# Funatiq/cuclark

Hardware: AMD Instinct MI355X
Metric: Mreads/sec (10M x 150bp, k=31) (higher is better)
Workload: dtype u64

## Files before the change

### cuclark_amd/_lib.py

```python
import ctypes as C
import importlib.util
import os
import subprocess

_PKG = os.path.dirname(os.path.abspath(__file__))
LIB_PATH = os.environ.get("MIC_LIB_PATH") or os.path.join(_PKG, "lib", "libmi_clark.so")
CSRC = os.path.join(_PKG, "csrc")

MIC_RESULT_WORDS = 8
MIC_FLAG_ROW_OVERFLOW = 1
MIC_FLAG_DENSE_PATH = 2
MIC_ROW_INVALID = 0xFFFFFFFF
MIC_ROLLUP_WORDS, MIC_ROLLUP_MAX_LEVELS = 8, 7
MIC_ROLLUP_UNRESOLVED, MIC_ROLLUP_PENDING = 0xFFFFFFFF, 0xFFFFFFFE
MIC_DENSITY_WORDS, MIC_DENSITY_CONF_BINS, MIC_DENSITY_GAMMA_BINS = 5153, 51, 101
MIC_KSKETCH_REGS = 16384
MIC_LAYOUT_AUTO, MIC_LAYOUT_DIRECT, MIC_LAYOUT_MINIMIZER, MIC_LAYOUT_SUPER, MIC_LAYOUT_SUPER2 = 0, 1, 2, 3, 4


class MicError(RuntimeError):
    def __init__(self, code, msg):
        super().__init__(f"libmi_clark error {code}: {msg}")
        self.code = code

# ... 63 lines not shown
    ("mic_batch_query_group", C.c_int, [C.POINTER(C.c_void_p), _SZ, _SZ, C.c_int]),
    ("mic_sync", C.c_int, [_VP]),
    ("mic_thread_bind_near_device", C.c_int, [_VP, C.c_int]),
    ("mic_batches_free", C.c_int, [_VP]),
    ("mic_query_device", C.c_int, [_VP, _VP, _VP, _SZ, _VP, _VP, _VP]),
    ("mic_resolve_flagged_device", C.c_int, [_VP, _VP, _VP, _VP, _VP, _VP, C.POINTER(_SZ)]),
    ("mic_merge_rows_device", C.c_int, [_VP, _VP, _VP, _VP, _SZ, _VP]),
    ("mic_result_from_rows_device", C.c_int, [_VP, _VP, _VP, _SZ, _VP]),
    ("mic_count_dense_device", C.c_int, [_VP, _VP, _VP, _VP, _SZ, _VP, _VP]),
    ("mic_result_from_dense_device", C.c_int, [_VP, _VP, _VP, _SZ, _VP, _VP, _VP]),
    ("mic_probe_stats_device", C.c_int, [_VP, _VP, _VP, _SZ, C.POINTER(C.c_uint64)]),
    ("mic_last_query_ms", C.c_int, [_VP, C.POINTER(C.c_float)]),
    ("mic_last_crowd_stats", C.c_int, [_VP, C.POINTER(C.c_uint32)]),
    ("mic_debug_fetch_crowd", C.c_int, [_VP, _VP, _SZ, C.POINTER(C.c_uint32)]),
    ("mic_debug_fetch_slots", C.c_int, [_VP, C.c_uint64, C.c_uint64, _VP]),
    ("mic_debug_stream_pool", C.c_int, [C.POINTER(C.c_uint32)]),
    ("mic_ingest_alloc", C.c_int, [_VP, _SZ, _SZ, C.POINTER(C.c_char_p), C.c_uint32, C.c_int, C.POINTER(_VP)]),
    ("mic_ingest_classify", C.c_int, [_VP, _SZ, _SZ, C.c_int, C.POINTER(MicIngestResult)]),
    ("mic_ingest_classify_group", C.c_int, [C.POINTER(C.c_void_p), _SZ, _SZ, _SZ, _SZ, C.c_int, C.POINTER(MicIngestResult)]),
    ("mic_ingest_fetch_group_rows", C.c_int, [_VP, _SZ, _SZ, _VP, _SZ, C.POINTER(C.c_uint64), C.POINTER(C.c_uint32)]),
    ("mic_ingest_group_stats", C.c_int, [_VP, C.POINTER(C.c_double), _SZ]),
    ("mic_ingest_fetch_packed", C.c_int, [_VP, _SZ, _VP, _SZ, _VP, _SZ, C.POINTER(C.c_uint64), C.POINTER(C.c_uint64)]),
    ("mic_ingest_free", C.c_int, [_VP]),
    ("mic_ingest_set_min_quality", C.c_int, [_VP, C.c_uint32]),
    ("mic_fastq_mask_quality", C.c_int, [_VP, _SZ, C.c_uint32, _VP]),
    ("mic_ingest_set_low_complexity", C.c_int, [_VP, C.c_uint32]),
    ("mic_text_mask_low_complexity", C.c_int, [_VP, _SZ, C.c_uint32, _VP]),
    ("mic_gz_inflate_device", C.c_int, [_VP, _VP, _SZ, C.POINTER(_VP), C.POINTER(_SZ), C.POINTER(C.c_uint32)]),
    ("mic_gz_copy_text", C.c_int, [_VP, _VP, _SZ, _SZ, _VP]),
    ("mic_gz_free_text", C.c_int, [_VP, _VP]),
# ... 141 lines not shown
```

### cuclark_amd/csrc/mic_build.hip

```cpp
#include "mic_internal.h"
#include "mic_device.h"

#include <stdio.h>
#include <stdlib.h>
#include <time.h>
#include <vector>
#include <math.h>

#include <hipcub/hipcub.hpp>

#define TILE 256

namespace {

struct TileA { unsigned long long elems; unsigned long long nonzero; };
struct TileB { unsigned long long ovf_slots; unsigned long long kept; unsigned int max_bucket; unsigned int pad; };

__device__ inline void block_scan2(uint32_t a, uint32_t b, uint32_t& ex_a, uint32_t& ex_b, uint32_t& tot_a,
                                   uint32_t& tot_b) {
  __shared__ uint32_t sa[TILE], sb[TILE];
  const int t = threadIdx.x;
  sa[t] = a; sb[t] = b;
  __syncthreads();
  for (int off = 1; off < TILE; off <<= 1) {
// ... 672 lines not shown
__device__ inline uint64_t s_x_of(unsigned long long K, uint32_t j, int k, int m) {
  return (K >> (2 * (k - m - (int)j))) & ((1ULL << (2 * m)) - 1);
}
__device__ inline bool s_less(unsigned long long Ka, uint32_t ma, unsigned long long Kb, uint32_t mb, int k, int m) {
  const uint64_t xa = s_x_of(Ka, ma & 0xFF, k, m), xb = s_x_of(Kb, mb & 0xFF, k, m);
  if ((uint32_t)xa != (uint32_t)xb) return (uint32_t)xa < (uint32_t)xb;
  if (xa != xb) return xa < xb;
  return (ma & 0xFF) < (mb & 0xFF);
}

struct SWriter {
  uint32_t* slots; uint64_t main, chain; uint32_t n_total, n_out;
  uint64_t cur, n_slots; uint32_t n_here, pool_cap; uint32_t* pool; bool full;
  uint32_t row[32];
  __device__ __forceinline__ void row_init() {
    row[0] = row[1] = row[2] = row[3] = row[4] = row[5] = 0xFFFFFFFFu;
    row[6] = row[7] = row[8] = row[9] = row[10] = row[11] = row[12] = row[13] = row[14] = row[15] = row[16] = row[17] = row[18] = 0;
    row[19] = row[20] = row[21] = row[22] = row[23] = row[24] = row[25] = row[26] = row[27] = row[28] = row[29] = row[30] = row[31] = 0;
  }
#define S_ROW_PUT(ee) { const bool h_ = e == ee; row[ee] = h_ ? key : row[ee]; row[6 + 3 * ee] = h_ ? a : row[6 + 3 * ee]; row[7 + 3 * ee] = h_ ? b : row[7 + 3 * ee]; \
                        row[8 + 3 * ee] = h_ ? c : row[8 + 3 * ee]; row[24 + ee] = h_ ? pl : row[24 + ee]; }
  __device__ __forceinline__ void put_main(uint32_t e, uint32_t key, uint32_t a, uint32_t b, uint32_t c, uint32_t pl) {
    static_assert(MIC_S_CAP == 6, "one S_ROW_PUT per entry of a slot");
    S_ROW_PUT(0) S_ROW_PUT(1) S_ROW_PUT(2) S_ROW_PUT(3) S_ROW_PUT(4) S_ROW_PUT(5)
  }
#undef S_ROW_PUT
  __device__ __forceinline__ void put(uint64_t slot, uint32_t e, uint32_t key, uint32_t a, uint32_t b, uint32_t c, uint32_t pl) {
    if (slot == main) put_main(e, key, a, b, c, pl);
    else { uint32_t* q = slots + slot * 32; q[e] = key; q[6 + 3 * e] = a; q[7 + 3 * e] = b; q[8 + 3 * e] = c; q[24 + e] = pl; }
  }
  __device__ __forceinline__ void set_hdr(uint64_t slot, uint32_t w30, uint32_t w31) {
    if (slot == main) { row[30] = w30; row[31] = w31; } else { uint32_t* q = slots + slot * 32; q[30] = w30; q[31] = w31; }
  }
};

__device__ inline void s_slot_init(uint32_t* q) {
  for (int e = 0; e < 6; ++e) q[e] = 0xFFFFFFFFu;
  for (int e = 6; e < 32; ++e) q[e] = 0;
}
template <int MODE>
__device__ __forceinline__ void s_emit(const SOpen& o, uint64_t x, int L, SWriter& wr) {
  const u128 v = o.S << (96 - 2 * L);
  const uint32_t v0 = (uint32_t)(v >> 64), v1 = (uint32_t)(v >> 32), v2 = (uint32_t)v, pl = (o.pmask << 16) | o.label;
  if (MODE == 2) {
    if (wr.n_here == MIC_S_CAP && !wr.full) {
      const uint32_t idx = atomicAdd(wr.pool, 1u);
      if (idx >= wr.pool_cap) { wr.full = true; atomicMax(wr.pool + 1, 1u); }
      else {
        const uint64_t nxt = wr.n_slots + idx;
        wr.set_hdr(wr.cur, MIC_S_CAP | MIC_S_NEXT, (uint32_t)nxt);
        s_slot_init(wr.slots + nxt * 32);
        wr.cur = nxt; wr.n_here = 0;
      }
    }
    if (!wr.full) wr.put(wr.cur, wr.n_here++, (uint32_t)x, v0, v1, v2, pl);
  }
  if (MODE == 1) {
    const uint32_t idx = wr.n_out, e = idx % MIC_S_CAP;
    if (idx < MIC_S_CAP) wr.put_main(e, (uint32_t)x, v0, v1, v2, pl);
    else { uint32_t* q = wr.slots + (wr.chain + (idx - MIC_S_CAP) / MIC_S_CAP) * 32; q[e] = (uint32_t)x; q[6 + 3 * e] = v0; q[7 + 3 * e] = v1; q[8 + 3 * e] = v2; q[24 + e] = pl; }
  }
  ++wr.n_out;
}

#define S_MAXOPEN 4
#define S_TPB 128
#define S_LDS_CAND 2048
template <int MODE>
__global__ void __launch_bounds__(S_TPB) s_merge_kernel(const unsigned long long* __restrict__ off, const uint32_t* __restrict__ cnt,
                                                        uint64_t n_slots, unsigned long long* __restrict__ cand_k,
                                                        uint32_t* __restrict__ cand_m, int k, int m,
                                                        uint32_t* __restrict__ n_ent, const unsigned long long* __restrict__ chain_off,
                                                        uint32_t* __restrict__ slots, uint32_t* __restrict__ max_ent,
                                                        uint64_t slot_lo, uint64_t slot_hi, unsigned long long base, int sort_now,
                                                        uint32_t* __restrict__ pool, uint32_t pool_cap) {
// ... 29 lines not shown
    kv = (r + 2 * m >= 64 ? 0ULL : left << (r + 2 * m)) | (x << r) | ((unsigned long long)F & ((1ULL << r) - 1));
  };
  const uint32_t n = live ? cnt[s] : 0;
  const unsigned long long my = live ? off[s] - base : c0;
  const int w = k - m + 1, L = k + w - 1;
  SWriter wr; wr.slots = slots; wr.main = s; wr.chain = 0; wr.n_total = 0; wr.n_out = 0;
  wr.cur = s; wr.n_slots = n_slots; wr.n_here = 0; wr.pool_cap = pool_cap; wr.pool = pool; wr.full = false;
  wr.row_init();
  if (WRITE && live) {
    wr.n_total = n_ent[s];
    const uint32_t n_chain = wr.n_total > MIC_S_CAP ? (wr.n_total - 1) / MIC_S_CAP : 0;
    wr.chain = n_slots + chain_off[s];
    for (uint32_t c = 0; c <= n_chain; ++c) {
      const uint32_t here = wr.n_total - c * MIC_S_CAP > MIC_S_CAP ? MIC_S_CAP : wr.n_total - c * MIC_S_CAP;
      const uint32_t w30 = (wr.n_total ? here : 0) | (c < n_chain ? MIC_S_NEXT : 0), w31 = c < n_chain ? (uint32_t)(wr.chain + c) : 0;
      if (c == 0) { wr.row[30] = w30; wr.row[31] = w31; }
      else { uint32_t* q = slots + (wr.chain + c - 1) * 32; s_slot_init(q); q[30] = w30; q[31] = w31; }
    }
  }
  auto sort_and_merge = [&](auto* K, auto* M) __attribute__((always_inline)) {
  if (sort_now) {
    constexpr uint32_t gaps[8] = {701, 301, 132, 57, 23, 10, 4, 1};
#pragma unroll
    for (int g = 0; g < 8; ++g) {
      const uint32_t gap = gaps[g];
      if (gap >= n) continue;
      for (uint32_t i = gap; i < n; ++i) {
        const unsigned long long kv = K[i]; const uint32_t mv = M[i];
        uint32_t j = i;
        while (j >= gap && (packed ? kv < K[j - gap] : s_less(kv, mv, K[j - gap], M[j - gap], k, m))) { K[j] = K[j - gap]; M[j] = M[j - gap]; j -= gap; }
        K[j] = kv; M[j] = mv;
      }
// ... 56 lines not shown
#undef S_ROW_OUT
  }
}

__global__ void s_chain_demand_kernel(const uint32_t* __restrict__ n_ent, uint64_t n, uint32_t* __restrict__ demand) {
  uint64_t i = (uint64_t)blockIdx.x * blockDim.x + threadIdx.x;
  if (i < n) { const uint32_t e = n_ent[i]; demand[i] = e > MIC_S_CAP ? (e - 1) / MIC_S_CAP : 0; }
}

#ifndef MIC_S_CROWD
#define MIC_S_CROWD 12
#endif

struct SChain {
  const uint32_t* slots; uint64_t slot; uint32_t e, n_here; bool valid;
  __device__ SChain(const uint32_t* sl, uint64_t s) : slots(sl), slot(s), e(0) { n_here = sl[s * 32 + 30] & 0xFFu; valid = true; settle(); }
  __device__ void settle() {
    while (valid && e >= n_here) {
      const uint32_t* q = slots + slot * 32;
      if (q[30] & MIC_S_NEXT) { slot = q[31]; n_here = slots[slot * 32 + 30] & 0xFFu; e = 0; } else valid = false;
    }
  }
  __device__ void next() { ++e; settle(); }
  __device__ const uint32_t* q() const { return slots + slot * 32; }
};

__device__ inline uint64_t s_entry_x(const uint32_t* q, uint32_t e, int k, int m) {
  const u128 S = ((u128)q[6 + 3 * e] << 64) | ((u128)q[7 + 3 * e] << 32) | q[8 + 3 * e];
  const int ctx = k - m;
  return (uint64_t)(S >> (96 - 2 * (ctx + m))) & ((1ULL << (2 * m)) - 1);
}

__global__ void __launch_bounds__(256) s_crowd_count_kernel(const uint32_t* __restrict__ slots, uint64_t slot_lo, uint64_t slot_hi, int k, int m,
                                                            unsigned long long* __restrict__ out) {
  const uint64_t s = slot_lo + (uint64_t)blockIdx.x * blockDim.x + threadIdx.x;
  if (s >= slot_hi) return;
  if ((slots[s * 32 + 30] & 0xFFu) < MIC_S_CAP || !(slots[s * 32 + 30] & MIC_S_NEXT)) return;
  SChain c(slots, s);
  while (c.valid) {
    const uint64_t x = s_entry_x(c.q(), c.e, k, m);
    uint32_t n = 0, kmers = 0;
    while (c.valid && s_entry_x(c.q(), c.e, k, m) == x) { ++n; kmers += __popc(c.q()[24 + c.e] >> 16); c.next(); }
    if (n > MIC_S_CROWD) { atomicAdd(&out[0], (unsigned long long)kmers); atomicAdd(&out[1], 1ull); }
  }
}

__device__ inline void s_side_insert(uint4* __restrict__ side, uint32_t mask, uint64_t K, uint32_t label1) {
  uint32_t h = s_side_hash(K, mask);
  for (;;) {
    uint32_t* cell = (uint32_t*)(side + h);
    if (atomicCAS(&cell[2], 0u, label1) == 0u) { cell[0] = (uint32_t)K; cell[1] = (uint32_t)(K >> 32); return; }
    h = (h + 1) & mask;
  }
}

__global__ void __launch_bounds__(256) s_crowd_move_kernel(uint32_t* __restrict__ slots, uint64_t slot_lo, uint64_t slot_hi, int k, int m,
                                                           uint4* __restrict__ side, uint32_t side_mask, uint32_t* __restrict__ n_ent,
                                                           uint32_t* __restrict__ max_ent) {
  const uint64_t s = slot_lo + (uint64_t)blockIdx.x * blockDim.x + threadIdx.x;
  if (s >= slot_hi) return;
  if ((slots[s * 32 + 30] & 0xFFu) < MIC_S_CAP || !(slots[s * 32 + 30] & MIC_S_NEXT)) return;
  {
    SChain c(slots, s);
    bool any = false;
    while (c.valid && !any) {
      const uint64_t x = s_entry_x(c.q(), c.e, k, m);
      uint32_t n = 0;
      while (c.valid && s_entry_x(c.q(), c.e, k, m) == x) { ++n; c.next(); }
      any = n > MIC_S_CROWD;
    }
    if (!any) return;
  }
  const int w = k - m + 1, ctx = k - m;
  SChain rd(slots, s);
  uint64_t w_slot = s; uint32_t w_e = 0, total = 0;
  auto put = [&](uint32_t key, uint32_t S0, uint32_t S1, uint32_t S2, uint32_t pl) {
    if (w_e == MIC_S_CAP) { w_slot = slots[w_slot * 32 + 31]; w_e = 0; }
    uint32_t* q = slots + w_slot * 32;
    q[w_e] = key; q[6 + 3 * w_e] = S0; q[7 + 3 * w_e] = S1; q[8 + 3 * w_e] = S2; q[24 + w_e] = pl;
    ++w_e; ++total;
  };
  while (rd.valid) {
    const uint64_t x = s_entry_x(rd.q(), rd.e, k, m);
    uint32_t n = 0;
    { SChain la = rd; while (la.valid && s_entry_x(la.q(), la.e, k, m) == x) { ++n; la.next(); } }
    if (n > MIC_S_CROWD) {
      for (uint32_t i = 0; i < n; ++i) {
        const uint32_t* q = rd.q();
        const uint32_t S0 = q[6 + 3 * rd.e], S1 = q[7 + 3 * rd.e], S2 = q[8 + 3 * rd.e], pl = q[24 + rd.e];
        for (int j = 0; j < w; ++j)
          if ((pl >> (16 + j)) & 1u) s_side_insert(side, side_mask, s_extract(S0, S1, S2, w - 1 - j, k), (pl & 0xFFFFu) + 1u);
        rd.next();
      }
      const u128 v = (u128)x << (96 - 2 * (ctx + m));
      put((uint32_t)x, (uint32_t)(v >> 64), (uint32_t)(v >> 32), (uint32_t)v, 0xFFFFu);
    } else {
      for (uint32_t i = 0; i < n; ++i) {
        const uint32_t* q = rd.q();
        const uint32_t key = q[rd.e], S0 = q[6 + 3 * rd.e], S1 = q[7 + 3 * rd.e], S2 = q[8 + 3 * rd.e], pl = q[24 + rd.e];
        rd.next();
        put(key, S0, S1, S2, pl);
      }
    }
  }
  {
    uint64_t sl = s; uint32_t left = total;
    for (;;) {
      uint32_t* q = slots + sl * 32;
      const uint32_t here = left > MIC_S_CAP ? MIC_S_CAP : left;
      left -= here;
      for (uint32_t e = here; e < MIC_S_CAP; ++e) { q[e] = 0xFFFFFFFFu; q[6 + 3 * e] = q[7 + 3 * e] = q[8 + 3 * e] = 0; q[24 + e] = 0; }
      const uint32_t nxt = q[31];
      if (left) { q[30] = here | MIC_S_NEXT; sl = nxt; } else { q[30] = here; q[31] = 0; break; }
    }
  }
  n_ent[s] = total;
  atomicMax(max_ent, total);
}

}

int mic_build_mtable(const uint8_t* d_sizes, uint64_t n_buckets, uint64_t bucket0, uint64_t htsize, const void* d_keys,
                     int key_bytes, const uint16_t* d_labels, uint32_t sampling, uint64_t rank_base, int k, int m,
                     hipStream_t s, MicBuildOut* out, char* err, size_t err_cap) {
  int rc = 0;
  const unsigned n_tiles = (unsigned)((n_buckets + TILE - 1) / TILE);
  TileA* d_a = nullptr; uint32_t* d_cnt = nullptr; uint32_t* d_cur = nullptr; unsigned long long* d_tile = nullptr;
  unsigned long long* d_kept = nullptr; uint32_t* d_max = nullptr; MSlot* slots = nullptr; uint32_t* d_of = nullptr;
// ... 598 lines not shown
```

### cuclark_amd/csrc/mic_device.h

```cpp
#ifndef MIC_DEVICE_H
#define MIC_DEVICE_H

#include "mic_internal.h"

__device__ __forceinline__ uint32_t bperm(int src_lane, uint32_t v) {
  return (uint32_t)__builtin_amdgcn_ds_bpermute(src_lane << 2, (int)v);
}

template <int CTRL>
__device__ __forceinline__ uint32_t quad_perm(uint32_t v) {
  return (uint32_t)__builtin_amdgcn_update_dpp(0, (int)v, CTRL, 0xF, 0xF, true);
}
#define QP_BCAST0 0x00
#define QP_BCAST1 0x55
#define QP_BCAST3 0xFF
#define QP_XOR1 0xB1
#define QP_XOR2 0x4E

__device__ __forceinline__ uint64_t revcomp_bits(uint64_t x, int k) {
  uint32_t rh = __builtin_bitreverse32((uint32_t)x), rl = __builtin_bitreverse32((uint32_t)(x >> 32));
  rh = ((rh >> 1) & 0x55555555u) | ((rh << 1) & ~0x55555555u);
  rl = ((rl >> 1) & 0x55555555u) | ((rl << 1) & ~0x55555555u);
  return (((uint64_t)~rh << 32) | (uint32_t)~rl) >> (64 - 2 * k);
}
// ... 36 lines not shown
#endif
}

__device__ __forceinline__ uint32_t mslot_of_kmer(uint64_t kmer, int k, int m, uint32_t n_slots) {
  const uint64_t mask = (1ULL << (2 * m)) - 1;
  uint32_t best = 0xFFFFFFFFu;
  for (int j = 0; j + m <= k; ++j) {
    uint32_t h = mmer_order_key((kmer >> (2 * (k - m - j))) & mask, m);
    best = h < best ? h : best;
  }
  return mslot_of_key(best, n_slots);
}

#define MIC_S_CAP 6
#define MIC_S_NEXT 0x100u

#ifndef MIC_S_MOD
#define MIC_S_MOD 1
#endif
__host__ __device__ __forceinline__ int s_tlen(int k, int m) {
  int t = m;
#if MIC_S_MOD
  const int w = k - m + 1;
  while (t - w >= 7) t -= w;
#endif
  return t;
}
__device__ __forceinline__ uint32_t s_torder(uint64_t tv) {
  uint32_t h = __umul24((uint32_t)tv & 0xFFFFFFu, 0x9E3779u) + 0x27D4EB2Fu;
  const uint32_t hi = (uint32_t)(tv >> 24);
// ... 129 lines not shown
    if (key < best) { best = key; bi = i; }
  }
  const int p = bi % w;
  const uint64_t mf = (K >> (2 * (k - m - p))) & mask;
  const uint64_t mr = fwd ? 0 : revcomp_bits(mf, m);
  const bool rev = !fwd && mr < mf;
  const uint64_t x = rev ? mr : mf;
  const uint64_t Kq = rev ? revcomp_bits(K, k) : K;
  const int j = rev ? w - 1 - p : p;
  uint64_t slot = sslot_of_x(x, n_slots);
  if (parted && (uint32_t)slot - slot_lo >= slot_cnt) { *mine = false; return 0; }
  *mine = true;
  for (;;) {
    const uint32_t* q = (const uint32_t*)(slots + slot * 8);
    for (int e = 0; e < MIC_S_CAP; ++e) {
      if (q[e] != (uint32_t)x) continue;
      const uint32_t pl = q[24 + e];
      if ((pl >> 16) == 0 && side && s_extract(q[6 + 3 * e], q[7 + 3 * e], q[8 + 3 * e], w - 1, m) == x) return s_side_probe(side, side_mask, Kq);
      if (!((pl >> (16 + j)) & 1)) continue;
      if (s_extract(q[6 + 3 * e], q[7 + 3 * e], q[8 + 3 * e], w - 1 - j, k) == Kq) return (pl & 0xFFFFu) + 1;
    }
    if (!(q[30] & MIC_S_NEXT)) return 0;
    slot = q[31];
  }
}

#define MIC_M_N(meta) ((meta) & 0xFFu)
#define MIC_M_DIR 0x100u

#endif
```

### cuclark_amd/csrc/mic_engine.hip

```cpp
#include "mi_clark.h"
#include "mic_internal.h"

#include <errno.h>
#include <stdarg.h>
#include <stdio.h>
#include <stdlib.h>
#include <string.h>
#include <time.h>

#include <sched.h>

#include <algorithm>
#include <mutex>
#include <string>
#include <atomic>
#include <thread>
#include <unistd.h>
#include <utility>
#include <vector>

static thread_local char g_err[512] = "";
thread_local uint64_t mic_build_reserved_hbm = 0;

namespace {
// ... 644 lines not shown
  if (e->slots) hipFree(e->slots);
  if (e->side) hipFree(e->side);
  if (e->d_sizes) hipFree(e->d_sizes);
  e->slots = nullptr; e->side = nullptr; e->d_sizes = nullptr; e->db_loaded = false;
  memset(&e->info, 0, sizeof(e->info));
  return MIC_OK;
}

int mic_db_get_info(const mic_engine* e, mic_db_info* info) {
  if (!e || !info) return mic_set_error(MIC_E_INVALID, "null argument");
  if (!e->db_loaded) return mic_set_error(MIC_E_STATE, "no database loaded");
  *info = e->info;
  return MIC_OK;
}

int mic_debug_fetch_slots(mic_engine* e, uint64_t first, uint64_t n, uint32_t* out) {
  if (!e || !out) return mic_set_error(MIC_E_INVALID, "null argument");
  if (!e->db_loaded) return mic_set_error(MIC_E_STATE, "no database loaded");
  if (e->table.layout != 2 || e->table.parted) return mic_set_error(MIC_E_UNSUPPORTED, "slots are fetched from a whole super-k-mer table only");
  if (first > e->info.n_slots || n > e->info.n_slots - first) return mic_set_error(MIC_E_INVALID, "slots [%llu, +%llu) of %llu",
                                                                                   (unsigned long long)first, (unsigned long long)n, (unsigned long long)e->info.n_slots);
  int rc = set_device(e);
  if (rc) return rc;
  MIC_TRY(hipDeviceSynchronize());
  if (n) MIC_TRY(hipMemcpy(out, e->table.slots + first * 8, n * 128, hipMemcpyDeviceToHost));
  return MIC_OK;
}

const char* mic_db_last_build_report(void) {
  static thread_local std::string copy;
  std::lock_guard<std::mutex> lk(g_report_mu);
  copy = g_report;
  return copy.c_str();
}

int mic_db_reserve_hbm(mic_engine* e, uint64_t bytes) {
  if (!e) return mic_set_error(MIC_E_INVALID, "null engine");
  e->reserve_hbm = bytes;
  return MIC_OK;
}

int mic_db_set_part(mic_engine* e, uint32_t part, uint32_t n_parts) {
// ... 742 lines not shown
```

### cuclark_amd/csrc/mic_kernels.hip

```cpp
#include "mic_internal.h"
#include "mic_device.h"
#include "mic_ksketch.h"
#include "mic_hitmap.h"
#include "mic_join2.h"

#include <stdlib.h>
#include <type_traits>

#ifndef MIC_EXP
#define MIC_EXP 0
#endif
#ifndef MIC_FUNNEL64
#define MIC_FUNNEL64 1
#endif
#ifndef MIC_X
#define MIC_X 0
#endif
#if MIC_X & 8
__device__ unsigned long long g_entry_walk[3];
extern "C" int mic_debug_entry_walk(unsigned long long out[3], int reset) {
  if (hipMemcpyFromSymbol(out, HIP_SYMBOL(g_entry_walk), sizeof(g_entry_walk)) != hipSuccess) return -1;
  const unsigned long long z[3] = {0, 0, 0};
  if (reset && hipMemcpyToSymbol(HIP_SYMBOL(g_entry_walk), z, sizeof(z)) != hipSuccess) return -1;
  return 0;
// ... 912 lines not shown
            for (int i = 0; i < MIC_RMAX / 8; ++i) sidx[i] = runslot[8 * i + (lane >> 3)];
#pragma unroll
            for (int i = 0; i < MIC_RMAX / 8; ++i) {
              if (8u * i >= nrun) break;
              if (8u * i + (lane >> 3) < nrun)
                __builtin_amdgcn_global_load_lds((const __attribute__((address_space(1))) void*)(slots + (uint64_t)sidx[i] * 8 + (lane & 7)),
                                                 (__attribute__((address_space(3))) void*)(stage + (64 + MIC_R_SKEW) * i), 16, 0, 0);
            }
            asm volatile("s_waitcnt vmcnt(0)" ::: "memory");
            __builtin_amdgcn_wave_barrier();
            {
              const bool v0 = s0_ != 0xFFFFFFFFu && rid0 - rbase < MIC_RMAX, v1 = s1_ != 0xFFFFFFFFu && rid1 - rbase < MIC_RMAX;
              const uint32_t* q0 = (const uint32_t*)(stage + (v0 ? staged_at(rid0 - rbase) : 0));
              const uint32_t* q1 = (const uint32_t*)(stage + (v1 ? staged_at(rid1 - rbase) : 0));
              const uint32_t t0 = tk32[0], t1 = tk32[1];
              uint32_t e0 = q0[3] < t0 ? 4u : 0u, e1 = q1[3] < t1 ? 4u : 0u;
              e0 += q0[e0 + 1] < t0 ? 2u : 0u; e1 += q1[e1 + 1] < t1 ? 2u : 0u;
              e0 += q0[e0 < 5 ? e0 : 5] < t0 ? 1u : 0u; e1 += q1[e1 < 5 ? e1 : 5] < t1 ? 1u : 0u;
              const uint32_t mz0 = q0[30], mz1 = q1[30];
              bool more0 = v0 && e0 < 6, more1 = v1 && e1 < 6;
              uint32_t hit0 = 0, hit1 = 0;
              e0 = e0 < 5 ? e0 : 5; e1 = e1 < 5 ? e1 : 5;
              for (;;) {
                const uint32_t g0 = q0[e0], g1 = q1[e1];
                const uint32_t a0 = q0[6 + 3 * e0], b0 = q0[7 + 3 * e0], c0 = q0[8 + 3 * e0], p0 = q0[24 + e0];
                const uint32_t a1 = q1[6 + 3 * e1], b1 = q1[7 + 3 * e1], c1 = q1[8 + 3 * e1], p1 = q1[24 + e1];
                const bool same0 = more0 && g0 == t0, same1 = more1 && g1 == t1;
                const bool m0 = same0 && ((p0 >> (16 + (w - 1) - ao[0])) & 1) && s_extract(a0, b0, c0, (int)ao[0], k) == ko[0];
                const bool m1 = same1 && ((p1 >> (16 + (w - 1) - ao[1])) & 1) && s_extract(a1, b1, c1, (int)ao[1], k) == ko[1];
                if (m0) hit0 = (p0 & 0xFFFFu) + 1;
                if (m1) hit1 = (p1 & 0xFFFFu) + 1;
                {
                  const bool cr0 = same0 && (p0 >> 16) == 0, cr1 = same1 && (p1 >> 16) == 0;
                  if (__ballot(cr0) | __ballot(cr1)) {
                    uint64_t kp = (uint64_t)__builtin_amdgcn_kernarg_segment_ptr();
                    asm volatile("" : "+s"(kp));
                    const __attribute__((address_space(4))) MicQueryArgs* kc = (const __attribute__((address_space(4))) MicQueryArgs*)kp;
                    const uint4* side = kc->t.side; const uint32_t smask = kc->t.side_mask;
                    const uint64_t mm = (1ULL << (2 * m)) - 1;
                    if (side && cr0 && s_extract(a0, b0, c0, w - 1, m) == ((ko[0] >> (2 * ao[0])) & mm)) hit0 = s_side_probe(side, smask, ko[0]);
                    if (side && cr1 && s_extract(a1, b1, c1, w - 1, m) == ((ko[1] >> (2 * ao[1])) & mm)) hit1 = s_side_probe(side, smask, ko[1]);
                  }
                }
                more0 = same0 && !m0 && e0 < 5; more1 = same1 && !m1 && e1 < 5;
                e0 += more0 ? 1u : 0u; e1 += more1 ? 1u : 0u;
                if (!(__ballot(more0) | __ballot(more1))) break;
              }
              if (v0) { o0_ = hit0; y0_ = 0xFFFFFFFFu; }
              if (v1) { o1_ = hit1; y1_ = 0xFFFFFFFFu; }
              const bool n0 = v0 && !hit0 && (mz0 & MIC_S_NEXT), n1 = v1 && !hit1 && (mz1 & MIC_S_NEXT);
              if (__ballot(n0) | __ballot(n1)) {
                if (n0 && q0[5] <= t0) y0_ = q0[31];
                if (n1 && q1[5] <= t1) y1_ = q1[31];
              }
            }
          }
        };
        while (__ballot(sl0 != 0xFFFFFFFFu) | __ballot(sl1 != 0xFFFFFFFFu)) {
          uint32_t nx0, nx1;
          level(sl0, sl1, res0, res1, nx0, nx1);
          sl0 = nx0; sl1 = nx1;
        }
        tally2(res0, res1, acc, n_ent, overflow, total, lane);
      }
    }
    uint32_t t_hdr, t_pp, t_pe;
    asm volatile("s_waitcnt vmcnt(0)" ::: "memory");
    __builtin_amdgcn_wave_barrier();
// ... 259 lines not shown
                                         (__attribute__((address_space(3))) void*)(uintptr_t)(so + 16u * (64 + MIC_R_SKEW) * (uint32_t)i), 16, 0, 0);
    }
  };
  auto consume = [&](Round& L, RowAcc& acc, uint32_t& n_ent, uint32_t& overflow, uint32_t& total, uint32_t& cg) __attribute__((always_inline)) {
    const uint32_t G0 = L.G0, G1 = L.G1, G2 = L.G2;
    uint32_t key, xhi_;
    region_x(G0, G1, key, xhi_);
    const int jmax = L.jmax, jmin = L.jmin;
    uint32_t cur = L.cur;
    int remaining = L.remaining;
    for (;;) {
      asm volatile("s_waitcnt vmcnt(0)" ::: "memory");
      __builtin_amdgcn_wave_barrier();
      const bool vl = cur != 0xFFFFFFFFu;
      const uint32_t* q = (const uint32_t*)(stage + (vl ? staged_at((uint32_t)lane) : 0));
      const uint4 ka = *(const uint4*)q;
      const uint2 kb = *(const uint2*)(q + 4);
      uint32_t e = (ka.x < key) + (ka.y < key) + (ka.z < key) + (ka.w < key) + (kb.x < key) + (kb.y < key);
      const uint32_t mz = q[30];
      const uint64_t m_vl = wballot(vl);
      uint64_t m_more = m_vl & wballot(e < 6), m_pos = 0;
      e = e < 5 ? e : 5;
#if MIC_X & 8
      uint32_t ew_pass = 0;
#endif
      for (;;) {
        uint32_t e3 = e + (e << 1);
        asm volatile("" : "+v"(e3));
        uint32_t g = q[e], g1 = q[e + 1], S0 = q[6 + e3], S1 = q[7 + e3], S2 = q[8 + e3], pl = q[24 + e];
        asm volatile("" : "+v"(S2));
        const uint64_t m_same = m_more & wballot(g == key);
        const uint64_t m_next = wballot(g1 == key);
        const uint32_t d0 = G0 ^ S0, d1 = G1 ^ S1, d2 = G2 ^ S2;
        const uint64_t m_hit = m_same & (k > 16
                                             ? wballot(((d0 & ((1u << ((32 - 2 * ctx) & 31)) - 1u)) | (d1 >> xsh)) == 0)
                                             : wballot((((((uint64_t)d0 << 32) | d1) << (2 * ctx)) >> (64 - 2 * m)) == 0));
        const uint32_t dl = d0 >> (32 - 2 * ctx);
        const uint32_t dr = k > 16 ? __builtin_amdgcn_alignbit(d1, d2, xsh)
                                        : (uint32_t)((((((uint64_t)d0 << 32) | d1)) << ((2 * k) & 63)) >> 32);
        const int left = __builtin_ctz(dl | (1u << (2 * ctx))) >> 1;
        const int right = __builtin_clz(dr | (1u << (31 - 2 * ctx))) >> 1;
        const int hi = left < jmax ? left : jmax, lo = ctx - right > jmin ? ctx - right : jmin;
        const uint32_t range = ((2u << (hi & 31)) - 1u) & (~0u << (lo & 31));
        const uint32_t hits = __builtin_amdgcn_inverse_ballot_w64(m_hit) ? (uint32_t)__popc((pl >> 16) & range) : 0u;
#if MIC_X & 8
// ... 15 lines not shown
        remaining -= (int)hits;
        m_pos = wballot(remaining > 0);
        m_more = m_same & m_pos & wballot(e < 5);
#if !(MIC_X & 256)
        m_more &= m_next;
#endif
        e += __builtin_amdgcn_inverse_ballot_w64(m_more) ? 1u : 0u;
        if (!m_more) break;
      }
#if MIC_X & 64
      break;
#endif
      const uint64_t m_nx = m_pos & wballot((mz & MIC_S_NEXT) != 0);
      if (!m_nx) break;
      cur = 0xFFFFFFFFu;
      if (__builtin_amdgcn_inverse_ballot_w64(m_nx) && q[5] <= key) cur = q[31];
      if (!wballot(cur != 0xFFFFFFFFu)) break;
      remaining = (cur == 0xFFFFFFFFu && remaining > 0) ? 0 : remaining;
      issue(cur, MIC_RMAX, lane_copy());
    }
    if (!(MIC_X & 2) && __builtin_expect(wballot(remaining <= MIC_R_CROWDED) != 0, 0)) {
      const bool crowded = remaining <= MIC_R_CROWDED;
      const uint32_t n_c = (uint32_t)__popcll(wballot(crowded));
      uint64_t kpv = (uint64_t)__builtin_amdgcn_kernarg_segment_ptr();
      asm volatile("" : "+v"(kpv));
      const MicQueryArgs* kv = (const MicQueryArgs*)kpv;
      uint32_t* cw = kv->crowd;
      uint32_t* itb = kv->crowd_items;
      const uint32_t icap = kv->crowd_item_cap;
      uint32_t ib = 0xFFFFFFFFu;
      if (cw != nullptr && cg != MIC_CG_DENSE) {
// ... 790 lines not shown
```

### cuclark_amd/db.py

```python
import ctypes as C

import numpy as np

from . import _lib
from ._lib import MicConfig, MicDbInfo, MicError, check, MIC_RESULT_WORDS


class MiClarkUnsupported(RuntimeError):
    """mic_gz_*: an input the device path does not take (MIC_E_UNSUPPORTED); the caller uses its other path."""


def _as_np(ptr, shape, dtype):
    n = int(np.prod(shape))
    if n == 0:
        return np.zeros(shape, dtype)
    buf = (C.c_char * (n * np.dtype(dtype).itemsize)).from_address(ptr)
    return np.frombuffer(buf, dtype=dtype).reshape(shape)


class MiClarkDB:
    def __init__(self, k, num_targets, num_batches=1, device=-1, row_words=16, layout=0):
        self.L = _lib.load()
        self.k = int(k)
        self.num_targets = int(num_targets)
# ... 483 lines not shown
                                            stream or None))

    def result_from_dense_device(self, d_counts, d_ids, n_ids, d_results, d_rows=0, stream=0):
        check(self.L.mic_result_from_dense_device(self.h, d_counts, d_ids or None, n_ids, d_results, d_rows or None, stream or None))

    def probe_stats_device(self, d_reads_pointer, d_containers, n_reads):
        out = (C.c_uint64 * 4)()
        check(self.L.mic_probe_stats_device(self.h, d_reads_pointer, d_containers, n_reads, out))
        return dict(kmers=int(out[0]), probed=int(out[1]), hits=int(out[2]), bucket_len_sum=int(out[3]))

    def last_query_ms(self):
        ms = C.c_float(0)
        check(self.L.mic_last_query_ms(self.h, C.byref(ms)))
        return float(ms.value)

    def fetch_slots(self, first=0, n=None):
        if n is None:
            n = int(self.info()["n_slots"]) - first
        out = np.empty((n, 32), np.uint32)
        check(self.L.mic_debug_fetch_slots(self.h, first, n, out.ctypes.data))
        return out

    def last_crowd_stats(self):
        out = (C.c_uint32 * 4)()
        check(self.L.mic_last_crowd_stats(self.h, out))
        return dict(reads=int(out[0]), runs=int(out[1]), row_words=int(out[2]), reads_to_dense_path=int(out[3]))
```

### include/mi_clark.h

```cpp
#ifndef MI_CLARK_H
#define MI_CLARK_H

#include <stddef.h>
#include <stdint.h>

#ifdef __cplusplus
extern "C" {
#endif

#define MIC_OK 0
#define MIC_E_INVALID (-1)
#define MIC_E_IO (-2)
#define MIC_E_NOMEM (-3)
#define MIC_E_HIP (-4)
#define MIC_E_STATE (-5)
#define MIC_E_NODEVICE (-6)
#define MIC_E_UNSUPPORTED (-7)

#define MIC_RESULT_WORDS 8
#define MIC_FLAG_ROW_OVERFLOW 1u
#define MIC_FLAG_DENSE_PATH 2u

#define MIC_ROW_INVALID 0xFFFFFFFFu
#define MIC_MAX_PART 65528u
// ... 83 lines not shown
                               uint32_t* d_results, uint32_t* d_rows, void* stream, size_t* n_resolved);
int mic_merge_rows_device(mic_engine* e, const uint32_t* d_rows_a, const uint32_t* d_rows_b, uint32_t* d_rows_out,
                          size_t n_reads, void* stream);
int mic_result_from_rows_device(mic_engine* e, const uint32_t* d_rows, uint32_t* d_results, size_t n_reads,
                                void* stream);
int mic_count_dense_device(mic_engine* e, const uint32_t* d_reads_pointer, const uint16_t* d_containers,
                           const uint32_t* d_read_ids, size_t n_ids, uint32_t* d_counts, void* stream);
int mic_result_from_dense_device(mic_engine* e, const uint32_t* d_counts, const uint32_t* d_ids, size_t n_ids,
                                 uint32_t* d_results, uint32_t* d_rows, void* stream);
int mic_probe_stats_device(mic_engine* e, const uint32_t* d_reads_pointer, const uint16_t* d_containers, size_t n_reads,
                           uint64_t out[4]);
int mic_last_query_ms(mic_engine* e, float* ms);
int mic_last_crowd_stats(mic_engine* e, uint32_t out[4]);
int mic_debug_fetch_crowd(mic_engine* e, uint32_t* out, size_t words, uint32_t caps[3]);
int mic_debug_fetch_slots(mic_engine* e, uint64_t first, uint64_t n, uint32_t* out);

#define MIC_INGEST_PAIRED 1
#define MIC_INGEST_FASTQ_2LINE 2
#define MIC_INGEST_RESIDENT 4
#define MIC_INGEST_RESIDENT_FASTQ 12
#define MIC_INGEST_NO_CSV 16
#define MIC_INGEST_OK 0u
#define MIC_INGEST_FALLBACK 1u
#define MIC_INGEST_ODD_RECORD 2u
#define MIC_INGEST_TRUNCATED 4u
#define MIC_INGEST_LONG_READ 8u
#define MIC_INGEST_TOO_MANY 16u
#define MIC_INGEST_DENSE 32u

typedef struct mic_ingest_result {
// ... 191 lines not shown
```

Before: 2363.

## Interleave super-k-mer slot entries so each entry loads as one 16-byte vector

Reorders the 32-word slot layout so each entry's three sequence words and payload sit together in an aligned 4-word group, with keys moved to words 24-29 and header/link at 30-31. Query kernels now fetch an entry with a single uint4 load and read keys, header and link through two vector loads instead of scattered scalar loads. The build writers, chain walkers and debug fetch are updated to the new layout, and a documented-layout conversion is added for debug output. Any external code that reads raw slots in the old layout would break.

```diff
diff --git a/cuclark_amd/_lib.py b/cuclark_amd/_lib.py
--- a/cuclark_amd/_lib.py
+++ b/cuclark_amd/_lib.py
@@ -101,6 +101,7 @@
     ("mic_last_crowd_stats", C.c_int, [_VP, C.POINTER(C.c_uint32)]),
     ("mic_debug_fetch_crowd", C.c_int, [_VP, _VP, _SZ, C.POINTER(C.c_uint32)]),
     ("mic_debug_fetch_slots", C.c_int, [_VP, C.c_uint64, C.c_uint64, _VP]),
+    ("mic_debug_fetch_slots_raw", C.c_int, [_VP, C.c_uint64, C.c_uint64, _VP]),
     ("mic_debug_stream_pool", C.c_int, [C.POINTER(C.c_uint32)]),
     ("mic_ingest_alloc", C.c_int, [_VP, _SZ, _SZ, C.POINTER(C.c_char_p), C.c_uint32, C.c_int, C.POINTER(_VP)]),
     ("mic_ingest_classify", C.c_int, [_VP, _SZ, _SZ, C.c_int, C.POINTER(MicIngestResult)]),
diff --git a/cuclark_amd/csrc/mic_build.hip b/cuclark_amd/csrc/mic_build.hip
--- a/cuclark_amd/csrc/mic_build.hip
+++ b/cuclark_amd/csrc/mic_build.hip
@@ -710,12 +710,13 @@
   uint64_t cur, n_slots; uint32_t n_here, pool_cap; uint32_t* pool; bool full;
   uint32_t row[32];
   __device__ __forceinline__ void row_init() {
-    row[0] = row[1] = row[2] = row[3] = row[4] = row[5] = 0xFFFFFFFFu;
-    row[6] = row[7] = row[8] = row[9] = row[10] = row[11] = row[12] = row[13] = row[14] = row[15] = row[16] = row[17] = row[18] = 0;
-    row[19] = row[20] = row[21] = row[22] = row[23] = row[24] = row[25] = row[26] = row[27] = row[28] = row[29] = row[30] = row[31] = 0;
-  }
-#define S_ROW_PUT(ee) { const bool h_ = e == ee; row[ee] = h_ ? key : row[ee]; row[6 + 3 * ee] = h_ ? a : row[6 + 3 * ee]; row[7 + 3 * ee] = h_ ? b : row[7 + 3 * ee]; \
-                        row[8 + 3 * ee] = h_ ? c : row[8 + 3 * ee]; row[24 + ee] = h_ ? pl : row[24 + ee]; }
+    static_assert(MIC_S_CAP == 6, "one s_entry_clear per entry of a slot");
+    s_entry_clear(row, 0); s_entry_clear(row, 1); s_entry_clear(row, 2); s_entry_clear(row, 3); s_entry_clear(row, 4); s_entry_clear(row, 5);
+    row[MIC_S_HDR] = row[MIC_S_LINK] = 0;
+  }
+#define S_ROW_PUT(ee) { const bool h_ = e == ee; row[MIC_S_KEY(ee)] = h_ ? key : row[MIC_S_KEY(ee)]; row[MIC_S_ENT(ee)] = h_ ? a : row[MIC_S_ENT(ee)]; \
+                        row[MIC_S_ENT(ee) + 1] = h_ ? b : row[MIC_S_ENT(ee) + 1]; row[MIC_S_ENT(ee) + 2] = h_ ? c : row[MIC_S_ENT(ee) + 2]; \
+                        row[MIC_S_PL(ee)] = h_ ? pl : row[MIC_S_PL(ee)]; }
   __device__ __forceinline__ void put_main(uint32_t e, uint32_t key, uint32_t a, uint32_t b, uint32_t c, uint32_t pl) {
     static_assert(MIC_S_CAP == 6, "one S_ROW_PUT per entry of a slot");
     S_ROW_PUT(0) S_ROW_PUT(1) S_ROW_PUT(2) S_ROW_PUT(3) S_ROW_PUT(4) S_ROW_PUT(5)
@@ -723,16 +724,16 @@
 #undef S_ROW_PUT
   __device__ __forceinline__ void put(uint64_t slot, uint32_t e, uint32_t key, uint32_t a, uint32_t b, uint32_t c, uint32_t pl) {
     if (slot == main) put_main(e, key, a, b, c, pl);
-    else { uint32_t* q = slots + slot * 32; q[e] = key; q[6 + 3 * e] = a; q[7 + 3 * e] = b; q[8 + 3 * e] = c; q[24 + e] = pl; }
+    else s_entry_put(slots + slot * 32, e, key, a, b, c, pl);
   }
   __device__ __forceinline__ void set_hdr(uint64_t slot, uint32_t w30, uint32_t w31) {
-    if (slot == main) { row[30] = w30; row[31] = w31; } else { uint32_t* q = slots + slot * 32; q[30] = w30; q[31] = w31; }
+    if (slot == main) { row[MIC_S_HDR] = w30; row[MIC_S_LINK] = w31; } else { uint32_t* q = slots + slot * 32; q[MIC_S_HDR] = w30; q[MIC_S_LINK] = w31; }
   }
 };
 
 __device__ inline void s_slot_init(uint32_t* q) {
-  for (int e = 0; e < 6; ++e) q[e] = 0xFFFFFFFFu;
-  for (int e = 6; e < 32; ++e) q[e] = 0;
+  for (uint32_t e = 0; e < MIC_S_CAP; ++e) s_entry_clear(q, e);
+  q[MIC_S_HDR] = q[MIC_S_LINK] = 0;
 }
 template <int MODE>
 __device__ __forceinline__ void s_emit(const SOpen& o, uint64_t x, int L, SWriter& wr) {
@@ -754,7 +755,7 @@
   if (MODE == 1) {
     const uint32_t idx = wr.n_out, e = idx % MIC_S_CAP;
     if (idx < MIC_S_CAP) wr.put_main(e, (uint32_t)x, v0, v1, v2, pl);
-    else { uint32_t* q = wr.slots + (wr.chain + (idx - MIC_S_CAP) / MIC_S_CAP) * 32; q[e] = (uint32_t)x; q[6 + 3 * e] = v0; q[7 + 3 * e] = v1; q[8 + 3 * e] = v2; q[24 + e] = pl; }
+    else s_entry_put(wr.slots + (wr.chain + (idx - MIC_S_CAP) / MIC_S_CAP) * 32, e, (uint32_t)x, v0, v1, v2, pl);
   }
   ++wr.n_out;
 }
@@ -814,8 +815,8 @@
     for (uint32_t c = 0; c <= n_chain; ++c) {
       const uint32_t here = wr.n_total - c * MIC_S_CAP > MIC_S_CAP ? MIC_S_CAP : wr.n_total - c * MIC_S_CAP;
       const uint32_t w30 = (wr.n_total ? here : 0) | (c < n_chain ? MIC_S_NEXT : 0), w31 = c < n_chain ? (uint32_t)(wr.chain + c) : 0;
-      if (c == 0) { wr.row[30] = w30; wr.row[31] = w31; }
-      else { uint32_t* q = slots + (wr.chain + c - 1) * 32; s_slot_init(q); q[30] = w30; q[31] = w31; }
+      if (c == 0) { wr.row[MIC_S_HDR] = w30; wr.row[MIC_S_LINK] = w31; }
+      else { uint32_t* q = slots + (wr.chain + c - 1) * 32; s_slot_init(q); q[MIC_S_HDR] = w30; q[MIC_S_LINK] = w31; }
     }
   }
   auto sort_and_merge = [&](auto* K, auto* M) __attribute__((always_inline)) {
@@ -902,11 +903,11 @@
 
 struct SChain {
   const uint32_t* slots; uint64_t slot; uint32_t e, n_here; bool valid;
-  __device__ SChain(const uint32_t* sl, uint64_t s) : slots(sl), slot(s), e(0) { n_here = sl[s * 32 + 30] & 0xFFu; valid = true; settle(); }
+  __device__ SChain(const uint32_t* sl, uint64_t s) : slots(sl), slot(s), e(0) { n_here = sl[s * 32 + MIC_S_HDR] & 0xFFu; valid = true; settle(); }
   __device__ void settle() {
     while (valid && e >= n_here) {
       const uint32_t* q = slots + slot * 32;
-      if (q[30] & MIC_S_NEXT) { slot = q[31]; n_here = slots[slot * 32 + 30] & 0xFFu; e = 0; } else valid = false;
+      if (q[MIC_S_HDR] & MIC_S_NEXT) { slot = q[MIC_S_LINK]; n_here = slots[slot * 32 + MIC_S_HDR] & 0xFFu; e = 0; } else valid = false;
     }
   }
   __device__ void next() { ++e; settle(); }
@@ -914,7 +915,7 @@
 };
 
 __device__ inline uint64_t s_entry_x(const uint32_t* q, uint32_t e, int k, int m) {
-  const u128 S = ((u128)q[6 + 3 * e] << 64) | ((u128)q[7 + 3 * e] << 32) | q[8 + 3 * e];
+  const u128 S = ((u128)q[MIC_S_ENT(e)] << 64) | ((u128)q[MIC_S_ENT(e) + 1] << 32) | q[MIC_S_ENT(e) + 2];
   const int ctx = k - m;
   return (uint64_t)(S >> (96 - 2 * (ctx + m))) & ((1ULL << (2 * m)) - 1);
 }
@@ -923,12 +924,12 @@
                                                             unsigned long long* __restrict__ out) {
   const uint64_t s = slot_lo + (uint64_t)blockIdx.x * blockDim.x + threadIdx.x;
   if (s >= slot_hi) return;
-  if ((slots[s * 32 + 30] & 0xFFu) < MIC_S_CAP || !(slots[s * 32 + 30] & MIC_S_NEXT)) return;
+  if ((slots[s * 32 + MIC_S_HDR] & 0xFFu) < MIC_S_CAP || !(slots[s * 32 + MIC_S_HDR] & MIC_S_NEXT)) return;
   SChain c(slots, s);
   while (c.valid) {
     const uint64_t x = s_entry_x(c.q(), c.e, k, m);
     uint32_t n = 0, kmers = 0;
-    while (c.valid && s_entry_x(c.q(), c.e, k, m) == x) { ++n; kmers += __popc(c.q()[24 + c.e] >> 16); c.next(); }
+    while (c.valid && s_entry_x(c.q(), c.e, k, m) == x) { ++n; kmers += __popc(c.q()[MIC_S_PL(c.e)] >> 16); c.next(); }
     if (n > MIC_S_CROWD) { atomicAdd(&out[0], (unsigned long long)kmers); atomicAdd(&out[1], 1ull); }
   }
 }
@@ -947,7 +948,7 @@
                                                            uint32_t* __restrict__ max_ent) {
   const uint64_t s = slot_lo + (uint64_t)blockIdx.x * blockDim.x + threadIdx.x;
   if (s >= slot_hi) return;
-  if ((slots[s * 32 + 30] & 0xFFu) < MIC_S_CAP || !(slots[s * 32 + 30] & MIC_S_NEXT)) return;
+  if ((slots[s * 32 + MIC_S_HDR] & 0xFFu) < MIC_S_CAP || !(slots[s * 32 + MIC_S_HDR] & MIC_S_NEXT)) return;
   {
     SChain c(slots, s);
     bool any = false;
@@ -963,9 +964,8 @@
   SChain rd(slots, s);
   uint64_t w_slot = s; uint32_t w_e = 0, total = 0;
   auto put = [&](uint32_t key, uint32_t S0, uint32_t S1, uint32_t S2, uint32_t pl) {
-    if (w_e == MIC_S_CAP) { w_slot = slots[w_slot * 32 + 31]; w_e = 0; }
-    uint32_t* q = slots + w_slot * 32;
-    q[w_e] = key; q[6 + 3 * w_e] = S0; q[7 + 3 * w_e] = S1; q[8 + 3 * w_e] = S2; q[24 + w_e] = pl;
+    if (w_e == MIC_S_CAP) { w_slot = slots[w_slot * 32 + MIC_S_LINK]; w_e = 0; }
+    s_entry_put(slots + w_slot * 32, w_e, key, S0, S1, S2, pl);
     ++w_e; ++total;
   };
   while (rd.valid) {
@@ -975,7 +975,7 @@
     if (n > MIC_S_CROWD) {
       for (uint32_t i = 0; i < n; ++i) {
         const uint32_t* q = rd.q();
-        const uint32_t S0 = q[6 + 3 * rd.e], S1 = q[7 + 3 * rd.e], S2 = q[8 + 3 * rd.e], pl = q[24 + rd.e];
+        const uint32_t S0 = q[MIC_S_ENT(rd.e)], S1 = q[MIC_S_ENT(rd.e) + 1], S2 = q[MIC_S_ENT(rd.e) + 2], pl = q[MIC_S_PL(rd.e)];
         for (int j = 0; j < w; ++j)
           if ((pl >> (16 + j)) & 1u) s_side_insert(side, side_mask, s_extract(S0, S1, S2, w - 1 - j, k), (pl & 0xFFFFu) + 1u);
         rd.next();
@@ -985,7 +985,7 @@
     } else {
       for (uint32_t i = 0; i < n; ++i) {
         const uint32_t* q = rd.q();
-        const uint32_t key = q[rd.e], S0 = q[6 + 3 * rd.e], S1 = q[7 + 3 * rd.e], S2 = q[8 + 3 * rd.e], pl = q[24 + rd.e];
+        const uint32_t key = q[MIC_S_KEY(rd.e)], S0 = q[MIC_S_ENT(rd.e)], S1 = q[MIC_S_ENT(rd.e) + 1], S2 = q[MIC_S_ENT(rd.e) + 2], pl = q[MIC_S_PL(rd.e)];
         rd.next();
         put(key, S0, S1, S2, pl);
       }
@@ -997,9 +997,9 @@
       uint32_t* q = slots + sl * 32;
       const uint32_t here = left > MIC_S_CAP ? MIC_S_CAP : left;
       left -= here;
-      for (uint32_t e = here; e < MIC_S_CAP; ++e) { q[e] = 0xFFFFFFFFu; q[6 + 3 * e] = q[7 + 3 * e] = q[8 + 3 * e] = 0; q[24 + e] = 0; }
-      const uint32_t nxt = q[31];
-      if (left) { q[30] = here | MIC_S_NEXT; sl = nxt; } else { q[30] = here; q[31] = 0; break; }
+      for (uint32_t e = here; e < MIC_S_CAP; ++e) s_entry_clear(q, e);
+      const uint32_t nxt = q[MIC_S_LINK];
+      if (left) { q[MIC_S_HDR] = here | MIC_S_NEXT; sl = nxt; } else { q[MIC_S_HDR] = here; q[MIC_S_LINK] = 0; break; }
     }
   }
   n_ent[s] = total;
diff --git a/cuclark_amd/csrc/mic_device.h b/cuclark_amd/csrc/mic_device.h
--- a/cuclark_amd/csrc/mic_device.h
+++ b/cuclark_amd/csrc/mic_device.h
@@ -74,6 +74,24 @@
 
 #define MIC_S_CAP 6
 #define MIC_S_NEXT 0x100u
+#define MIC_S_ENT(e) (4 * (e))
+#define MIC_S_PL(e) (4 * (e) + 3)
+#define MIC_S_KEY(e) (24 + (e))
+#define MIC_S_KEYS 24
+#define MIC_S_HDR 30
+#define MIC_S_LINK 31
+__host__ __device__ __forceinline__ void s_entry_put(uint32_t* q, uint32_t e, uint32_t key, uint32_t S0, uint32_t S1, uint32_t S2, uint32_t pl) {
+  q[MIC_S_KEY(e)] = key; q[MIC_S_ENT(e)] = S0; q[MIC_S_ENT(e) + 1] = S1; q[MIC_S_ENT(e) + 2] = S2; q[MIC_S_PL(e)] = pl;
+}
+__host__ __device__ __forceinline__ void s_entry_clear(uint32_t* q, uint32_t e) { s_entry_put(q, e, 0xFFFFFFFFu, 0, 0, 0, 0); }
+inline void s_slot_to_documented(const uint32_t* raw, uint32_t* out) {
+  for (uint32_t e = 0; e < MIC_S_CAP; ++e) {
+    out[e] = raw[MIC_S_KEY(e)];
+    out[6 + 3 * e] = raw[MIC_S_ENT(e)]; out[7 + 3 * e] = raw[MIC_S_ENT(e) + 1]; out[8 + 3 * e] = raw[MIC_S_ENT(e) + 2];
+    out[24 + e] = raw[MIC_S_PL(e)];
+  }
+  out[30] = raw[MIC_S_HDR]; out[31] = raw[MIC_S_LINK];
+}
 
 #ifndef MIC_S_MOD
 #define MIC_S_MOD 1
@@ -233,14 +251,15 @@
   for (;;) {
     const uint32_t* q = (const uint32_t*)(slots + slot * 8);
     for (int e = 0; e < MIC_S_CAP; ++e) {
-      if (q[e] != (uint32_t)x) continue;
-      const uint32_t pl = q[24 + e];
-      if ((pl >> 16) == 0 && side && s_extract(q[6 + 3 * e], q[7 + 3 * e], q[8 + 3 * e], w - 1, m) == x) return s_side_probe(side, side_mask, Kq);
+      if (q[MIC_S_KEY(e)] != (uint32_t)x) continue;
+      const uint4 en = slots[slot * 8 + MIC_S_ENT(e) / 4];
+      const uint32_t pl = en.w;
+      if ((pl >> 16) == 0 && side && s_extract(en.x, en.y, en.z, w - 1, m) == x) return s_side_probe(side, side_mask, Kq);
       if (!((pl >> (16 + j)) & 1)) continue;
-      if (s_extract(q[6 + 3 * e], q[7 + 3 * e], q[8 + 3 * e], w - 1 - j, k) == Kq) return (pl & 0xFFFFu) + 1;
+      if (s_extract(en.x, en.y, en.z, w - 1 - j, k) == Kq) return (pl & 0xFFFFu) + 1;
     }
-    if (!(q[30] & MIC_S_NEXT)) return 0;
-    slot = q[31];
+    if (!(q[MIC_S_HDR] & MIC_S_NEXT)) return 0;
+    slot = q[MIC_S_LINK];
   }
 }
 
diff --git a/cuclark_amd/csrc/mic_engine.hip b/cuclark_amd/csrc/mic_engine.hip
--- a/cuclark_amd/csrc/mic_engine.hip
+++ b/cuclark_amd/csrc/mic_engine.hip
@@ -1,5 +1,6 @@
 #include "mi_clark.h"
 #include "mic_internal.h"
+#include "mic_device.h"
 
 #include <errno.h>
 #include <stdarg.h>
@@ -682,7 +683,7 @@
   return MIC_OK;
 }
 
-int mic_debug_fetch_slots(mic_engine* e, uint64_t first, uint64_t n, uint32_t* out) {
+static int fetch_slots(mic_engine* e, uint64_t first, uint64_t n, uint32_t* out, bool documented) {
   if (!e || !out) return mic_set_error(MIC_E_INVALID, "null argument");
   if (!e->db_loaded) return mic_set_error(MIC_E_STATE, "no database loaded");
   if (e->table.layout != 2 || e->table.parted) return mic_set_error(MIC_E_UNSUPPORTED, "slots are fetched from a whole super-k-mer table only");
@@ -692,8 +693,16 @@
   if (rc) return rc;
   MIC_TRY(hipDeviceSynchronize());
   if (n) MIC_TRY(hipMemcpy(out, e->table.slots + first * 8, n * 128, hipMemcpyDeviceToHost));
-  return MIC_OK;
-}
+  if (documented)
+    for (uint64_t i = 0; i < n; ++i) {
+      uint32_t raw[32];
+      memcpy(raw, out + i * 32, sizeof raw);
+      s_slot_to_documented(raw, out + i * 32);
+    }
+  return MIC_OK;
+}
+int mic_debug_fetch_slots(mic_engine* e, uint64_t first, uint64_t n, uint32_t* out) { return fetch_slots(e, first, n, out, true); }
+int mic_debug_fetch_slots_raw(mic_engine* e, uint64_t first, uint64_t n, uint32_t* out) { return fetch_slots(e, first, n, out, false); }
 
 const char* mic_db_last_build_report(void) {
   static thread_local std::string copy;
diff --git a/cuclark_amd/csrc/mic_kernels.hip b/cuclark_amd/csrc/mic_kernels.hip
--- a/cuclark_amd/csrc/mic_kernels.hip
+++ b/cuclark_amd/csrc/mic_kernels.hip
@@ -950,17 +950,18 @@
               const uint32_t* q0 = (const uint32_t*)(stage + (v0 ? staged_at(rid0 - rbase) : 0));
               const uint32_t* q1 = (const uint32_t*)(stage + (v1 ? staged_at(rid1 - rbase) : 0));
               const uint32_t t0 = tk32[0], t1 = tk32[1];
-              uint32_t e0 = q0[3] < t0 ? 4u : 0u, e1 = q1[3] < t1 ? 4u : 0u;
-              e0 += q0[e0 + 1] < t0 ? 2u : 0u; e1 += q1[e1 + 1] < t1 ? 2u : 0u;
-              e0 += q0[e0 < 5 ? e0 : 5] < t0 ? 1u : 0u; e1 += q1[e1 < 5 ? e1 : 5] < t1 ? 1u : 0u;
-              const uint32_t mz0 = q0[30], mz1 = q1[30];
+              uint32_t e0 = q0[MIC_S_KEY(3)] < t0 ? 4u : 0u, e1 = q1[MIC_S_KEY(3)] < t1 ? 4u : 0u;
+              e0 += q0[MIC_S_KEY(e0 + 1)] < t0 ? 2u : 0u; e1 += q1[MIC_S_KEY(e1 + 1)] < t1 ? 2u : 0u;
+              e0 += q0[MIC_S_KEY(e0 < 5 ? e0 : 5)] < t0 ? 1u : 0u; e1 += q1[MIC_S_KEY(e1 < 5 ? e1 : 5)] < t1 ? 1u : 0u;
+              const uint32_t mz0 = q0[MIC_S_HDR], mz1 = q1[MIC_S_HDR];
               bool more0 = v0 && e0 < 6, more1 = v1 && e1 < 6;
               uint32_t hit0 = 0, hit1 = 0;
               e0 = e0 < 5 ? e0 : 5; e1 = e1 < 5 ? e1 : 5;
               for (;;) {
-                const uint32_t g0 = q0[e0], g1 = q1[e1];
-                const uint32_t a0 = q0[6 + 3 * e0], b0 = q0[7 + 3 * e0], c0 = q0[8 + 3 * e0], p0 = q0[24 + e0];
-                const uint32_t a1 = q1[6 + 3 * e1], b1 = q1[7 + 3 * e1], c1 = q1[8 + 3 * e1], p1 = q1[24 + e1];
+                const uint32_t g0 = q0[MIC_S_KEY(e0)], g1 = q1[MIC_S_KEY(e1)];
+                const uint4 en0 = *(const uint4*)(q0 + MIC_S_ENT(e0)), en1 = *(const uint4*)(q1 + MIC_S_ENT(e1));
+                const uint32_t a0 = en0.x, b0 = en0.y, c0 = en0.z, p0 = en0.w;
+                const uint32_t a1 = en1.x, b1 = en1.y, c1 = en1.z, p1 = en1.w;
                 const bool same0 = more0 && g0 == t0, same1 = more1 && g1 == t1;
                 const bool m0 = same0 && ((p0 >> (16 + (w - 1) - ao[0])) & 1) && s_extract(a0, b0, c0, (int)ao[0], k) == ko[0];
                 const bool m1 = same1 && ((p1 >> (16 + (w - 1) - ao[1])) & 1) && s_extract(a1, b1, c1, (int)ao[1], k) == ko[1];
@@ -986,8 +987,8 @@
               if (v1) { o1_ = hit1; y1_ = 0xFFFFFFFFu; }
               const bool n0 = v0 && !hit0 && (mz0 & MIC_S_NEXT), n1 = v1 && !hit1 && (mz1 & MIC_S_NEXT);
               if (__ballot(n0) | __ballot(n1)) {
-                if (n0 && q0[5] <= t0) y0_ = q0[31];
-                if (n1 && q1[5] <= t1) y1_ = q1[31];
+                if (n0 && q0[MIC_S_KEY(5)] <= t0) y0_ = q0[MIC_S_LINK];
+                if (n1 && q1[MIC_S_KEY(5)] <= t1) y1_ = q1[MIC_S_LINK];
               }
             }
           }
@@ -1277,10 +1278,10 @@
       __builtin_amdgcn_wave_barrier();
       const bool vl = cur != 0xFFFFFFFFu;
       const uint32_t* q = (const uint32_t*)(stage + (vl ? staged_at((uint32_t)lane) : 0));
-      const uint4 ka = *(const uint4*)q;
-      const uint2 kb = *(const uint2*)(q + 4);
+      const uint4 ka = *(const uint4*)(q + MIC_S_KEYS);
+      const uint4 kb = *(const uint4*)(q + MIC_S_KEYS + 4);
       uint32_t e = (ka.x < key) + (ka.y < key) + (ka.z < key) + (ka.w < key) + (kb.x < key) + (kb.y < key);
-      const uint32_t mz = q[30];
+      const uint32_t mz = kb.z;
       const uint64_t m_vl = wballot(vl);
       uint64_t m_more = m_vl & wballot(e < 6), m_pos = 0;
       e = e < 5 ? e : 5;
@@ -1288,10 +1289,10 @@
       uint32_t ew_pass = 0;
 #endif
       for (;;) {
-        uint32_t e3 = e + (e << 1);
-        asm volatile("" : "+v"(e3));
-        uint32_t g = q[e], g1 = q[e + 1], S0 = q[6 + e3], S1 = q[7 + e3], S2 = q[8 + e3], pl = q[24 + e];
-        asm volatile("" : "+v"(S2));
+        typedef uint32_t entry_words __attribute__((ext_vector_type(4)));
+        entry_words en = *(const entry_words*)(q + MIC_S_ENT(e));
+        asm volatile("" : "+v"(en));
+        uint32_t g = q[MIC_S_KEY(e)], g1 = q[MIC_S_KEY(e) + 1], S0 = en.x, S1 = en.y, S2 = en.z, pl = en.w;
         const uint64_t m_same = m_more & wballot(g == key);
         const uint64_t m_next = wballot(g1 == key);
         const uint32_t d0 = G0 ^ S0, d1 = G1 ^ S1, d2 = G2 ^ S2;
@@ -1337,7 +1338,7 @@
       const uint64_t m_nx = m_pos & wballot((mz & MIC_S_NEXT) != 0);
       if (!m_nx) break;
       cur = 0xFFFFFFFFu;
-      if (__builtin_amdgcn_inverse_ballot_w64(m_nx) && q[5] <= key) cur = q[31];
+      if (__builtin_amdgcn_inverse_ballot_w64(m_nx) && kb.y <= key) cur = kb.w;
       if (!wballot(cur != 0xFFFFFFFFu)) break;
       remaining = (cur == 0xFFFFFFFFu && remaining > 0) ? 0 : remaining;
       issue(cur, MIC_RMAX, lane_copy());
diff --git a/cuclark_amd/db.py b/cuclark_amd/db.py
--- a/cuclark_amd/db.py
+++ b/cuclark_amd/db.py
@@ -521,11 +521,11 @@
         check(self.L.mic_last_query_ms(self.h, C.byref(ms)))
         return float(ms.value)
 
-    def fetch_slots(self, first=0, n=None):
+    def fetch_slots(self, first=0, n=None, raw=False):
         if n is None:
             n = int(self.info()["n_slots"]) - first
         out = np.empty((n, 32), np.uint32)
-        check(self.L.mic_debug_fetch_slots(self.h, first, n, out.ctypes.data))
+        check((self.L.mic_debug_fetch_slots_raw if raw else self.L.mic_debug_fetch_slots)(self.h, first, n, out.ctypes.data))
         return out
 
     def last_crowd_stats(self):
diff --git a/include/mi_clark.h b/include/mi_clark.h
--- a/include/mi_clark.h
+++ b/include/mi_clark.h
@@ -121,6 +121,7 @@
 int mic_last_crowd_stats(mic_engine* e, uint32_t out[4]);
 int mic_debug_fetch_crowd(mic_engine* e, uint32_t* out, size_t words, uint32_t caps[3]);
 int mic_debug_fetch_slots(mic_engine* e, uint64_t first, uint64_t n, uint32_t* out);
+int mic_debug_fetch_slots_raw(mic_engine* e, uint64_t first, uint64_t n, uint32_t* out);
 
 #define MIC_INGEST_PAIRED 1
 #define MIC_INGEST_FASTQ_2LINE 2
```

Result: no change. 2380 (median of 6 runs) (+0.7%).
